# lpastura/kubernetes-1

Measured on AMD Instinct MI355X. Metric: pods scheduled/sec, higher is better.
Workload: dtype int64; 1 GPU; (b) 5000 nodes / 1913000 pods; nodes=5000, nodes_per_gpu=5000, pods=1913000, percentage_of_nodes_to_score=100, parallelism=1 GPU

## Files before the change

### kubernetes-1_amd/csrc/kgpu_kernels.hip

```cpp
#include <hip/hip_runtime.h>

#include <algorithm>
#include <map>
#include <mutex>
#include <tuple>

#include "kgpu_internal.h"

#if defined(__HIP_DEVICE_COMPILE__)
#define GAS __attribute__((address_space(1)))
#define CAS __attribute__((address_space(4)))
#else
#define GAS
#define CAS
#endif

namespace kgpu {

template <class T>
__device__ __forceinline__ GAS T* gp(T* p) {
  return (GAS T*)p;
}
template <class T>
__device__ __forceinline__ const CAS T* cp(const T* p) {
  return (const CAS T*)p;
}


constexpr uint32_t kRuntime = 0xFFFFFFFFu;
constexpr uint32_t kDefRes = 1u << 31;
constexpr uint32_t kSMask = (1u << KGPU_NUM_SCORES) - 1;

__device__ __forceinline__ uint64_t splitmix64(uint64_t x) {
  x += 0x9E3779B97F4A7C15ull;
  uint64_t z = x;
  z = (z ^ (z >> 30)) * 0xBF58476D1CE4E5B9ull;
  z = (z ^ (z >> 27)) * 0x94D049BB133111EBull;
  return z ^ (z >> 31);
}
__device__ __forceinline__ uint64_t pod_tie_key(uint64_t seed, int64_t seq) {
  return splitmix64(seed ^ ((uint64_t)seq * 0x9E3779B97F4A7C15ull));
}
__device__ __forceinline__ uint64_t rank40(uint64_t k, uint64_t idx, int mode) {
  if (mode == 1) return kMask40 - idx;
  uint64_t x = idx & kMask40;
  x ^= k & kMask40;
  x = (x * 0xD6E8FEB865ull) & kMask40;
  x ^= x >> 19;
  x = (x * 0x94D049BB13ull) & kMask40;
  x ^= x >> 23;
  x ^= (k >> 24) & kMask40;
  return x;
}

__device__ __forceinline__ uint64_t rank40_inv(uint64_t k, uint64_t x, int mode) {
  if (mode == 1) return kMask40 - x;
  x ^= (k >> 24) & kMask40;
  x ^= x >> 23;
  x = (x * 0x38E12D471Bull) & kMask40;
  x ^= (x >> 19) ^ (x >> 38);
  x = (x * 0xB38E39396Dull) & kMask40;
  x ^= k & kMask40;
  return x;
}

__device__ __forceinline__ bool list_has(const int32_t* v, int n, int x) {
  for (int i = 0; i < n; ++i)
    if (cp(v)[i] == x) return true;
  return false;
}

__device__ bool node_req(const DevState& st, const kgpu_req& r, int n) {
  const int v = r.key >= 0 ? gp(st.label_val)[(size_t)r.key * st.N + n] : -1;
  switch (r.op) {
    case KGPU_OP_IN:
      return v >= 0 && list_has(st.qp.ints + r.vals.begin, r.vals.count, v);
    case KGPU_OP_NOTIN:
      return v < 0 || !list_has(st.qp.ints + r.vals.begin, r.vals.count, v);
    case KGPU_OP_EXISTS:
      return v >= 0;
    case KGPU_OP_DNE:
      return v < 0;
    default: {
      if (v < 0) return false;
      const int idx = gp(st.value_off)[r.key] + v;
      if (!gp(st.value_int_ok)[idx]) return false;
      const int64_t lv = gp(st.value_int)[idx];
      return r.op == KGPU_OP_GT ? lv > r.imm : lv < r.imm;
    }
  }
}

__device__ bool node_reqs_all(const DevState& st, kgpu_range rr, int n) {
  for (int i = 0; i < rr.count; ++i)
    if (!node_req(st, cp(st.qp.reqs)[rr.begin + i], n)) return false;
  return true;
}

__device__ bool node_affinity_ok(const DevState& st, const kgpu_pod_query& q, int n) {
  if (!node_reqs_all(st, q.node_selector, n)) return false;
  if (!(q.flags & KGPU_Q_REQ_NODE_AFFINITY)) return true;
  const int g = st.node_base + n;
  for (int t = 0; t < q.req_terms.count; ++t) {
    const kgpu_node_term term = cp(st.qp.node_terms)[q.req_terms.begin + t];
    if (term.never_match) continue;
    if (!node_reqs_all(st, term.reqs, n)) continue;
    if (term.field_op == KGPU_OP_IN && g != term.field_node) continue;
    if (term.field_op == KGPU_OP_NOTIN && g == term.field_node) continue;
    return true;
  }
  return false;
}

struct NodeRes {
  int64_t ac, am, ae;
  int64_t rc, rm, re;
  int64_t zc, zm;
  int32_t ap, np;
  double ic, im;
};

__device__ __forceinline__ NodeRes load_res(const DevState& st, int n) {
  NodeRes r;
  r.ac = gp(st.alloc_cpu)[n]; r.am = gp(st.alloc_mem)[n]; r.ae = gp(st.alloc_eph)[n];
  r.rc = gp(st.req_cpu)[n]; r.rm = gp(st.req_mem)[n]; r.re = gp(st.req_eph)[n];
  r.zc = gp(st.nz_cpu)[n]; r.zm = gp(st.nz_mem)[n];
  r.ap = gp(st.alloc_pods)[n]; r.np = gp(st.num_pods)[n];
  r.ic = 0.0;
  r.im = 0.0;
  return r;
}

__device__ __forceinline__ void set_recips(NodeRes& r) {
  r.ic = (r.ac > 0 && r.ac < (1ll << 52)) ? 1.0 / (double)r.ac : 0.0;
  r.im = (r.am > 0 && r.am < (1ll << 52)) ? 1.0 / (double)r.am : 0.0;
}

__device__ __forceinline__ uint32_t fit_detail(const DevState& st, const kgpu_pod_query& q, const NodeRes& r, int n) {
  uint32_t d = 0;
  if (r.np + 1 > r.ap) d |= 1u;
  if (q.flags & KGPU_Q_FIT_ALL_ZERO) return d;
  if (r.ac < q.req[0] + r.rc) d |= 2u;
  if (r.am < q.req[1] + r.rm) d |= 4u;
  if (r.ae < q.req[2] + r.re) d |= 8u;
  for (int i = 0; i < q.scalars.count; ++i) {
    const kgpu_scalar_req s = cp(st.qp.scalars)[q.scalars.begin + i];
    if (!s.check) continue;
    const int64_t alloc = s.col >= 0 ? gp(st.alloc_scalar)[(size_t)s.col * st.N + n] : 0;
    const int64_t used = s.col >= 0 ? gp(st.req_scalar)[(size_t)s.col * st.N + n] : 0;
    if (alloc < s.value + used) d |= 16u << (i < 11 ? i : 11);
  }
  return d;
}

__device__ __forceinline__ bool ports_conflict(const DevState& st, const kgpu_pod_query& q, int n) {
  const int have = gp(st.port_count)[n];
  for (int i = 0; i < q.ports.count; ++i) {
    const kgpu_port w = cp(st.qp.ports)[q.ports.begin + i];
// ... 1042 lines not shown
        __hip_atomic_fetch_or(abort_word, kAbortDirty, __ATOMIC_RELAXED, __HIP_MEMORY_SCOPE_AGENT);
        return;
      }
    }
  }
}
__device__ __forceinline__ void lds_wait(int* f, int v, int32_t* abort_word) { lds_wait_t<false>(f, v, abort_word); }
__device__ __forceinline__ void lds_wait_ge(int* f, int v, int32_t* abort_word) { lds_wait_t<true>(f, v, abort_word); }

__device__ __forceinline__ constexpr bool spare_slot(int j, int K, int tid, int B) {
  return j == K - 1 && tid == B - 1;
}

template <int K, int B>
__device__ __forceinline__ void wg_partials(BatchShared<B>& sh, int p, const uint64_t (&keys)[K], bool vb, int ob,
                                            int jb, int cand, Cand& ra, Cand& rb) {
  const int tid = threadIdx.x, lane = tid & 63, wave = tid >> 6;
  Cand a{0, -1, 0}, b{0, -1, 0};
  if (!vb) {
#pragma unroll
    for (int j = 0; j < K; ++j) {
      const uint64_t k = spare_slot(j, K, tid, B) ? 0 : keys[j];
      a.feas += __popcll(__ballot(k != 0));
      if (k > a.key) { a.key = k; a.idx = j * B + tid; }
    }
    wave_argmax(a.key, a.idx);
  } else {
    uint64_t m = 0, kc = 0, ks = 0;
    int mi = -1, f0 = 0;
#pragma unroll
    for (int j = 0; j < K; ++j) {
      const bool spare = spare_slot(j, K, tid, B), isc = tid == ob && j == jb;
      const uint64_t k = (spare || isc) ? 0 : keys[j];
      f0 += __popcll(__ballot(k != 0));
      if (k > m) { m = k; mi = j * B + tid; }
      if (isc) kc = keys[j];
      if (spare) ks = keys[j];
    }
    wave_argmax(m, mi);
    const uint64_t kcu = (ob >> 6) == wave ? (uint64_t)lane64((int64_t)kc, ob & 63) : 0;
    const uint64_t ksu = ((B - 1) >> 6) == wave ? (uint64_t)lane64((int64_t)ks, (B - 1) & 63) : 0;
    a = Cand{m, mi, f0 + (kcu != 0 ? 1 : 0)};
    if (kcu > m) { a.key = kcu; a.idx = jb * B + ob; }
    b = Cand{m, mi, f0 + (ksu != 0 ? 1 : 0)};
    if (ksu > m) { b.key = ksu; b.idx = cand; }
  }
  if (lane == 0) {
    sh.ka[p][wave] = a.key; sh.ia[p][wave] = a.idx; sh.fa[p][wave] = a.feas;
    sh.kb[p][wave] = b.key; sh.ib[p][wave] = b.idx; sh.fb[p][wave] = b.feas;
  }
  ra = a;
  rb = b;
}

template <int B>
__device__ __forceinline__ Cand wg_combine(const BatchShared<B>& sh, int p, bool variant_b) {
  Cand c{0, -1, 0};
#pragma unroll
  for (int w = 0; w < B / 64; ++w) {
    const uint64_t k = variant_b ? sh.kb[p][w] : sh.ka[p][w];
    const int i = variant_b ? sh.ib[p][w] : sh.ia[p][w];
    c.feas += variant_b ? sh.fb[p][w] : sh.fa[p][w];
    if (k > c.key) { c.key = k; c.idx = i; }
  }
  return c;
}

template <int K, int B>
__device__ __forceinline__ Cand wave_recombine(const BatchShared<B>& sh, int p, const uint64_t (&keys)[K]) {
  const int tid = threadIdx.x, wave = tid >> 6;
  Cand a{0, -1, 0};
#pragma unroll
  for (int j = 0; j < K; ++j) {
    const uint64_t k = spare_slot(j, K, tid, B) ? 0 : keys[j];
    a.feas += __popcll(__ballot(k != 0));
    if (k > a.key) { a.key = k; a.idx = j * B + tid; }
  }
  wave_argmax(a.key, a.idx);
  Cand c{0, -1, 0};
#pragma unroll
  for (int w = 0; w < B / 64; ++w) {
    const bool me = w == wave;
    const uint64_t k = me ? a.key : sh.ka[p][w];
    const int i = me ? a.idx : sh.ia[p][w];
    c.feas += me ? a.feas : sh.fa[p][w];
    if (k > c.key) { c.key = k; c.idx = i; }
  }
  return c;
}

template <int NJ>
struct Sweep {
  uint64_t v[NJ];
  int abort;
};
template <int NJ, bool SYS>
__device__ __forceinline__ Sweep<NJ> sweep(const uint64_t* row, int G, const int32_t* abort_word, uint64_t fill) {
  const int lane = threadIdx.x & 63;
  Sweep<NJ> s;
#pragma unroll
  for (int j = 0; j < NJ; ++j) {
    uint64_t* p = const_cast<uint64_t*>(row + lane + 64 * j);
    s.v[j] = (lane + 64 * j < G) ? (SYS ? __hip_atomic_load(p, __ATOMIC_RELAXED, __HIP_MEMORY_SCOPE_SYSTEM) : load_sc1(p))
                                 : fill;
  }
  s.abort = load_sc1(abort_word);
  return s;
}

template <int NJ>
__device__ __forceinline__ bool row_done(const Sweep<NJ>& cur, uint64_t tmask, uint64_t expect, uint64_t& wkey,
                                         int& wg) {
  const int lane = threadIdx.x & 63;
  bool all = true;
  uint64_t k = 0;
  int gsel = -1;
#pragma unroll
  for (int j = 0; j < NJ; ++j) {
    const uint64_t v = cur.v[j];
    if ((v & tmask) != expect) {
      all = false;
    } else if ((v & ~tmask) > k) {
      k = v & ~tmask;
      gsel = lane + 64 * j;
    }
  }
  if (!__all(all)) return false;
  wave_argmax(k, gsel);
  wkey = k;
  wg = k ? gsel : -1;
  return true;
}
template <int NJ, bool SYS>
__device__ __forceinline__ bool poll_row(const uint64_t* row, int G, const int32_t* abort_word, uint64_t tmask,
                                         uint64_t expect, uint64_t& wkey, int& wg) {
  const uint64_t t0 = __builtin_amdgcn_s_memrealtime();
  Sweep<NJ> a = sweep<NJ, SYS>(row, G, abort_word, expect);
  for (;;) {
    const Sweep<NJ> b = sweep<NJ, SYS>(row, G, abort_word, expect);
    if (a.abort != 0) return false;
    if (row_done<NJ>(a, tmask, expect, wkey, wg)) return true;
    a = sweep<NJ, SYS>(row, G, abort_word, expect);
    if (b.abort != 0) return false;
    if (row_done<NJ>(b, tmask, expect, wkey, wg)) return true;
    if (__builtin_amdgcn_s_memrealtime() - t0 > kSpinTimeout) return false;
  }
}

struct HRow {
  int64_t ac, am, zc, zm;
  double ic, im;
};

template <uint32_t FM, uint32_t SM, int K, int B, bool XG, bool HB = false>
__global__ __launch_bounds__(B + 64 + (HB ? 2 * B : 0)) void k_batch(const DevState* __restrict__ stp, BatchArgs pa) {
  static_assert(!HB || (B == 64 && !XG &&
                       SM == ((1u << KGPU_S_BALANCED_ALLOCATION) | (1u << KGPU_S_LEAST_ALLOCATED) | kDefRes)),
                "the helper wave splits config (b)'s profile on the one-row-wave geometry");
  const DevState& st = *stp;
  constexpr int W = B / 64;
  const int tid = threadIdx.x, wave = tid >> 6, lane = tid & 63;
  const int G = gridDim.x, g = blockIdx.x;
  if (g == pa.hold) return;
  const int lo = g * pa.per;
  const int GT = pa.GT, gme = pa.rank * G + g;
  constexpr bool xg = XG;
  const uint64_t tmask = xg ? (0xFull << 60) : kGValid;
  __shared__ BatchShared<B> sh;
  __shared__ int64_t sh_hk[HB ? 2 * 2 * K * B : 1];
  __shared__ int sh_hready[2];
  __shared__ uint64_t* sh_peer_g[XG ? kMaxRanks : 1];
  __shared__ int32_t* sh_peer_f[XG ? kMaxRanks : 1];
  if constexpr (XG) {
    if (wave == W && lane < pa.nranks) {
      sh_peer_g[lane] = pa.pgran[lane];
      sh_peer_f[lane] = pa.pfeas[lane];
    }
  }
  if (tid == 0) {
    sh.bready = 0;
    sh.cready = 0;
    sh_hready[0] = 0;
    sh_hready[1] = 0;
  }
  __syncthreads();
  auto ring_row = [&](int k) -> size_t { return xg ? (size_t)((pa.xseq0 + k) % pa.R) : (size_t)k; };
  auto ring_tag = [&](int k) -> uint64_t {
    return xg ? (kGValid | ((uint64_t)(((pa.xseq0 + k) / pa.R) & 7) << 60)) : kGValid;
  };
  auto publish = [&](int i, uint64_t key, int feas) {
    const size_t roff = ring_row(i) * GT + gme;
    const uint64_t gtag = ring_tag(i);
    if constexpr (!XG) {
      store_sc1(pa.gran + roff, gtag | key);
      pa.feas[roff] = feas;
    } else {
      for (int rk = 0; rk < pa.nranks; ++rk) {
        __hip_atomic_store(sh_peer_g[rk] + roff, gtag | key, __ATOMIC_RELAXED, __HIP_MEMORY_SCOPE_SYSTEM);
        __hip_atomic_store(sh_peer_f[rk] + roff, feas, __ATOMIC_RELAXED, __HIP_MEMORY_SCOPE_SYSTEM);
      }
    }
  };
  const bool tr = pa.trace && (g == 0 || g == G - 1);
  int64_t* trow = pa.trace ? pa.trace + (g == 0 ? 0 : 8) : nullptr;
#define KGPU_STAMP(i, k) \
  if (tr && (tid == 0 || tid == B)) trow[(size_t)(i) * 16 + (k)] = (int64_t)__builtin_amdgcn_s_memrealtime()

  if constexpr (HB) {
    if (wave == W + 1 || wave == W + 2) {
      const int hw = wave - W - 1;
      HRow h[K];
#pragma unroll
      for (int j = 0; j < K; ++j) {
        const int n = lo + j * B + lane;
        h[j] = HRow{0, 0, 0, 0, 0.0, 0.0};
        if (!spare_slot(j, K, lane, B) && n < st.N) {
          h[j].ac = gp(st.alloc_cpu)[n];
          h[j].am = gp(st.alloc_mem)[n];
          h[j].zc = gp(st.nz_cpu)[n];
          h[j].zm = gp(st.nz_mem)[n];
          h[j].ic = (h[j].ac > 0 && h[j].ac < (1ll << 52)) ? 1.0 / (double)h[j].ac : 0.0;
          h[j].im = (h[j].am > 0 && h[j].am < (1ll << 52)) ? 1.0 / (double)h[j].am : 0.0;
        }
      }
      __builtin_amdgcn_s_waitcnt(0);
      const int64_t wl = st.w_of[KGPU_S_LEAST_ALLOCATED], wbal = st.w_of[KGPU_S_BALANCED_ALLOCATION];
      int cand = -1;
      bool staged = false;
      for (int i = 0; i <= pa.count; ++i) {
        const bool have_prev = i > 0, have_cur = i < pa.count;
        const int p = i & 1;
        const kgpu_pod_query* qc = st.queries + pa.first + i;
        const kgpu_pod_query* qpp = st.queries + pa.first + i - 1;
        const bool qmem = have_prev && (cp(qpp)->scalars.count | cp(qpp)->ports.count) != 0;
        const bool fast_b = have_prev && cand >= 0 && staged && pa.assume && !qmem;
        const int ob = cand >= 0 ? cand % B : -1, jb = cand >= 0 ? cand / B : -1;
        if (have_cur) {
          if (fast_b) {
            HRow t{};
#pragma unroll
            for (int j = 0; j < K; ++j)
              if (j == jb) {
                t.ac = lane64(h[j].ac, ob);
                t.am = lane64(h[j].am, ob);
                t.zc = lane64(h[j].zc, ob) + cp(qpp)->nz[0];
                t.zm = lane64(h[j].zm, ob) + cp(qpp)->nz[1];
                t.ic = __builtin_bit_cast(double, lane64(__builtin_bit_cast(int64_t, h[j].ic), ob));
                t.im = __builtin_bit_cast(double, lane64(__builtin_bit_cast(int64_t, h[j].im), ob));
              }
            if (lane == B - 1) h[K - 1] = t;
          }
          kgpu_pod_query qh;
          qh.score_req[0] = cp(qc)->score_req[0];
          qh.score_req[1] = cp(qc)->score_req[1];
#pragma unroll
          for (int j = 0; j < K; ++j) {
            const bool spare = spare_slot(j, K, lane, B);
            const int n = spare ? lo + cand : lo + j * B + lane;
            NodeRes nr{};
            nr.ac = h[j].ac; nr.am = h[j].am; nr.zc = h[j].zc; nr.zm = h[j].zm; nr.ic = h[j].ic; nr.im = h[j].im;
            sh_hk[((hw * 2 + p) * K + j) * B + lane] =
                hw == 0 ? least_score<true>(st, qh, nr, n) * wl : balanced_score(qh, nr) * wbal;
          }
          if (lane == 0) lds_release(&sh_hready[hw], i + 1);
        }
        __syncthreads();
        int wg = -1;
        if (have_prev) {
          if (sh.rabort[(i - 1) & 1]) break;
          wg = sh.rwg[(i - 1) & 1];
        }
        const bool won = have_prev && wg == gme;
        if (won && pa.assume && lane == ob) {
#pragma unroll
          for (int j = 0; j < K; ++j)
            if (j == jb) {
              h[j].zc += cp(qpp)->nz[0];
              h[j].zm += cp(qpp)->nz[1];
            }
        }
        const bool slow = have_cur && won && pa.assume && !fast_b;
        int cn = -1;
        if (have_cur && !slow) {
          const Cand c = wg_combine<B>(sh, p, won && fast_b);
          cn = c.key ? c.idx : -1;
        }
        if (slow) {
          lds_wait(&sh.cready, i + 1, pa.abort);
          cand = sh.cslow[p];
        } else {
          cand = cn;
        }
        staged = have_cur && !slow && cand >= 0;
      }
      return;
    }
  }
  if (wave == W) {
    constexpr int kQWords = (int)(sizeof(kgpu_pod_query) / 8);
    static_assert(kQWords <= 64, "one query row per prefetch instruction");
    int cand = -1;
    bool staged = false;
    for (int i = 0; i <= pa.count; ++i) {
      const bool have_prev = i > 0, have_cur = i < pa.count;
      const int p = i & 1;
      if (i == pa.abort_at && g == 0 && lane == 0) __hip_atomic_store(pa.abort, 1, __ATOMIC_RELAXED, __HIP_MEMORY_SCOPE_AGENT);
      if (i + 2 < pa.count) {
        const uint64_t v = lane < kQWords ? reinterpret_cast<const uint64_t*>(st.queries + pa.first + i + 2)[lane] : 0;
        asm volatile("" ::"v"(v));
      }
      bool qmem = false;
      if (have_prev) {
        const kgpu_pod_query* qq = st.queries + pa.first + i - 1;
        qmem = (cp(qq)->scalars.count | cp(qq)->ports.count) != 0;
      }
      const bool fast_b = have_prev && cand >= 0 && staged && pa.assume && !qmem;
      uint64_t wkey = 0;
      int wg = -1;
      bool ok = true;
      if (have_prev) {
        const uint64_t* prow = pa.gran + ring_row(i - 1) * GT;
        const uint64_t expect = ring_tag(i - 1);
        if constexpr (!XG)
          ok = poll_row<4, false>(prow, GT, pa.abort, tmask, expect, wkey, wg);
        else if (GT <= 256)
          ok = poll_row<4, true>(prow, GT, pa.abort, tmask, expect, wkey, wg);
        else
          ok = poll_row<16, true>(prow, GT, pa.abort, tmask, expect, wkey, wg);
        KGPU_STAMP(i, 7);
      }
      const bool won = have_prev && wg == gme;
      const bool slow = have_cur && won && pa.assume && !fast_b;
      if (ok) {
        if (have_prev && lane == 0 && (xg ? g == 0 : (won || (wg < 0 && g == 0)))) {
          kgpu_result res;
          res.node = wg < 0 ? -1
                   : xg ? (int32_t)rank40_inv(pod_tie_key(st.seed, pa.seq0 + i - 1), wkey & kMask40, st.tie_mode)
                        : st.node_base + lo + cand;
          res.feasible = 0;
          res.evaluated = st.n_total;
          res.scored = 0;
          res.score = wg >= 0 ? (int64_t)(wkey >> 40) - 1 : 0;
          gp(st.results)[pa.first + i - 1] = res;
        }
      } else if (lane == 0) {
        __hip_atomic_fetch_or(pa.abort, (i <= 1 && !XG) ? kAbortClean : kAbortDirty, __ATOMIC_RELAXED,
                              __HIP_MEMORY_SCOPE_AGENT);
      }
      if (lane == 0 && have_prev) {
        sh.rwg[(i - 1) & 1] = wg;
        sh.rabort[(i - 1) & 1] = ok ? 0 : 1;
      }
      __syncthreads();
      if (!ok) break;
      int cn = -1;
      if (have_cur && !slow) {
        KGPU_STAMP(i, 6);
        const Cand c = wg_combine<B>(sh, p, won && fast_b);
        if (lane == 0) publish(i, c.key, c.feas);
        KGPU_STAMP(i, 3);
        cn = c.key ? c.idx : -1;
      }
      if (slow) {
        lds_wait(&sh.cready, i + 1, pa.abort);
        cand = sh.cslow[p];
      } else {
        cand = cn;
      }
      staged = have_cur && !slow && cand >= 0;
    }
    return;
  }

  constexpr bool kStream = K > 4;
  constexpr int KR = kStream ? 1 : K;
  static_assert(!kStream || (W > 1 && !HB), "streamed rows: the candidate row travels through sh.brow");
  constexpr bool kRecip = (SM & kDefRes) != 0 && SM != kRuntime;
  NodeRes r[KR];
#pragma unroll
  for (int j = 0; j < KR; ++j) {
    const int n = lo + j * B + tid;
    r[j] = NodeRes{};
    if (!kStream && !spare_slot(j, K, tid, B) && n < st.N) r[j] = load_row<kRecip>(st, n);
  }
  __builtin_amdgcn_s_waitcnt(0);

  kgpu_pod_query qp{};
  kgpu_pod_query q = *cp(st.queries + pa.first);
  int cand = -1;
  bool staged = false;
  for (int i = 0; i <= pa.count; ++i) {
    KGPU_STAMP(i, 0);
    const bool have_prev = i > 0;
    const bool have_cur = i < pa.count;
    const int p = i & 1;
    const bool fast_b = have_prev && cand >= 0 && staged && pa.assume && qp.scalars.count == 0 && qp.ports.count == 0;
    const int ob = cand >= 0 ? cand % B : -1, jb = cand >= 0 ? cand / B : -1;
    uint64_t keys[K];
    Cand own_a{0, -1, 0}, own_b{0, -1, 0};
    if (have_cur) {
      const uint64_t tk = pod_tie_key(st.seed, pa.seq0 + i);
      if (fast_b && wave == W - 1) {
        NodeRes t;
        if constexpr (W == 1) {
#pragma unroll
          for (int j = 0; j < K; ++j)
            if (j == jb) t = lane_row(r[j], ob);
        } else {
          lds_wait(&sh.bready, i, pa.abort);
          t = sh.brow[(i - 1) & 1];
        }
        assume_regs(qp, t);
        if (tid == B - 1) r[KR - 1] = t;
      }
      if constexpr (HB) {
        uint32_t fs[K];
        uint64_t rkj[K];
#pragma unroll
        for (int j = 0; j < K; ++j) {
          const bool spare = spare_slot(j, K, tid, B);
          const int n = spare ? lo + cand : lo + j * B + tid;
          fs[j] = (spare ? fast_b : n < st.N) ? run_filters<FM>(st, q, r[j], n) : 1u;
          rkj[j] = rank40(tk, (uint64_t)(st.node_base + n), st.tie_mode);
        }
        if (q.scalars.count | q.ports.count) vm_drain();
        lds_wait_ge(&sh_hready[0], i + 1, pa.abort);
        lds_wait_ge(&sh_hready[1], i + 1, pa.abort);
#pragma unroll
        for (int j = 0; j < K; ++j) {
          const int64_t tot = sh_hk[((0 * 2 + p) * K + j) * B + tid] + sh_hk[((1 * 2 + p) * K + j) * B + tid];
          keys[j] = fs[j] ? 0 : (((uint64_t)(tot + 1) << 40) | rkj[j]);
        }
      } else {
#pragma unroll
        for (int j = 0; j < K; ++j) {
          const bool spare = spare_slot(j, K, tid, B);
          const int n = spare ? lo + cand : lo + j * B + tid;
          if constexpr (kStream) {
            const bool live = spare ? fast_b : n < st.N;
            NodeRes rj = r[0];
            if (!spare && live) rj = load_row<kRecip>(st, n);
            keys[j] = live ? node_key<FM, SM>(st, q, rj, n, tk) : 0;
          } else {
            keys[j] = (spare ? fast_b : n < st.N) ? node_key<FM, SM>(st, q, r[j], n, tk) : 0;
          }
        }
      }
      KGPU_STAMP(i, 5);
      wg_partials<K, B>(sh, p, keys, fast_b, ob, jb, cand, own_a, own_b);
    }
    KGPU_STAMP(i, 1);
    kgpu_pod_query qn{};
    if (i + 1 < pa.count) qn = *cp(st.queries + pa.first + i + 1);
    __syncthreads();
    KGPU_STAMP(i, 2);
    int wg = -1;
    if (have_prev) {
      const int s = (i - 1) & 1;
      if (sh.rabort[s]) break;
      wg = sh.rwg[s];
    }
    const bool won = have_prev && wg == gme;
    int cn = -1;
    if (have_cur) {
      if (won && pa.assume && !fast_b) {
        cn = -2;
      } else {
        const Cand c = W == 1 ? ((won && fast_b) ? own_b : own_a) : wg_combine<B>(sh, p, won && fast_b);
        cn = c.key ? c.idx : -1;
      }
    }
    if (won && pa.assume && tid == ob) {
#pragma unroll
      for (int j = 0; j < K; ++j)
        if (j == jb) {
          if constexpr (kStream) {
            NodeRes t = load_res(st, lo + (j * B + tid));
            assume_row(st, qp, t, lo + (j * B + tid));
          } else {
            assume_row(st, qp, r[j], lo + (j * B + tid));
          }
          assume_counts(st, pa.first + i - 1, lo + (j * B + tid));
        }
    }
    const bool slow = cn == -2;
    if (slow) {
      if (wave == ob / 64) {
        if (tid == ob) {
          const uint64_t tk = pod_tie_key(st.seed, pa.seq0 + i);
#pragma unroll
          for (int j = 0; j < K; ++j)
            if (j == jb) {
              if constexpr (kStream) keys[j] = node_key<FM, SM>(st, q, load_row<kRecip>(st, lo + (j * B + tid)), lo + (j * B + tid), tk);
              else keys[j] = node_key<FM, SM>(st, q, r[j], lo + (j * B + tid), tk);
            }
        }
        const Cand c = wave_recombine<K, B>(sh, p, keys);
        if (lane == 0) {
          publish(i, c.key, c.feas);
          sh.cslow[p] = c.key ? c.idx : -1;
          lds_release(&sh.cready, i + 1);
        }
      }
      lds_wait(&sh.cready, i + 1, pa.abort);
      cand = sh.cslow[p];
    } else {
      cand = cn;
      if (W > 1 && cand >= 0 && tid == cand % B) {
#pragma unroll
        for (int j = 0; j < K; ++j)
          if (j == cand / B) {
            if constexpr (kStream) sh.brow[p] = load_row<kRecip>(st, lo + cand);
            else sh.brow[p] = r[j];
          }
        if (i != pa.skip_release_at) lds_release(&sh.bready, i + 1);
      }
    }
    staged = have_cur && !slow && cand >= 0;
    qp = q;
    q = qn;
    KGPU_STAMP(i, 4);
  }
#undef KGPU_STAMP
}

__global__ __launch_bounds__(256) void k_batch_fixup(const DevState* __restrict__ stp, BatchArgs pa, int G) {
  const DevState& st = *stp;
  const int lane = threadIdx.x & 63;
  const int i = blockIdx.x * 4 + (threadIdx.x >> 6);
  for (int64_t z = (int64_t)blockIdx.x * blockDim.x + threadIdx.x; z < pa.zero_n16; z += (int64_t)gridDim.x * blockDim.x) {
    uint4* zp = reinterpret_cast<uint4*>(pa.zero_buf) + z;
    *zp = uint4{0, 0, 0, 0};
  }
  if (pa.abort_out && blockIdx.x == 0 && threadIdx.x == 0)
    __hip_atomic_store(pa.abort_out, load_sc1(pa.abort), __ATOMIC_RELAXED, __HIP_MEMORY_SCOPE_SYSTEM);
  if (i >= pa.count) return;
  const size_t row = pa.R > 0 ? (size_t)((pa.xseq0 + i) % pa.R) : (size_t)i;
  int f = 0;
  for (int g = lane; g < pa.GT; g += 64) f += pa.feas[row * pa.GT + g];
  f = (int)wave_sum32((uint32_t)f);
  (void)G;
  if (lane == 0) {
    kgpu_result& r = gp(st.results)[pa.first + i];
    r.feasible = f;
    if (r.node >= 0 && f >= 2) {
      r.scored = 1;
    } else {
      r.scored = 0;
      r.score = 0;
    }
    if (pa.res_out) pa.res_out[pa.first + i] = r;
  }
}

__device__ __forceinline__ int nval(const DevState& st, int k, int n) {
  return k >= 0 ? gp(st.label_val)[(size_t)k * st.N + n] : -1;
}
__device__ __forceinline__ int64_t* slot_ptr(const DevState& st, const QPlan& pl, int slot) {
  return st.scratch + pl.slot_off[slot];
}
__device__ __forceinline__ TopoHdr* hdr(const DevState& st) { return reinterpret_cast<TopoHdr*>(st.scratch); }
__device__ __forceinline__ int64_t* zone_sums(const DevState& st) { return st.scratch + kHdrWords; }
__device__ __forceinline__ void add64(int64_t* p, int64_t v) {
  atomicAdd(reinterpret_cast<unsigned long long*>(p), (unsigned long long)v);
}
__device__ __forceinline__ unsigned long long enc_max(int64_t x) { return (unsigned long long)x ^ (1ull << 63); }
__device__ __forceinline__ void amax64(int64_t* p, int64_t x) {
  atomicMax(reinterpret_cast<unsigned long long*>(p), enc_max(x));
}
__device__ __forceinline__ void amin64(int64_t* p, int64_t x) {
  atomicMax(reinterpret_cast<unsigned long long*>(p), ~enc_max(x));
}
__device__ __forceinline__ int64_t read_max(const int64_t* p) {
  const unsigned long long u = *reinterpret_cast<const unsigned long long*>(p);
  return u ? (int64_t)(u ^ (1ull << 63)) : INT64_MIN;
}
__device__ __forceinline__ int64_t read_min(const int64_t* p) {
  const unsigned long long u = *reinterpret_cast<const unsigned long long*>(p);
  return u ? (int64_t)(~u ^ (1ull << 63)) : INT64_MAX;
}

__device__ __forceinline__ bool all_keys(const DevState& st, const TSpread* c, int nc, int n) {
  for (int i = 0; i < nc; ++i)
    if (nval(st, c[i].key, n) < 0) return false;
  return true;
}

__device__ uint32_t topo_filter(int f, const DevState& st, const QPlan& pl, int n) {
  const TopoHdr* h = hdr(st);
  if (f == KGPU_F_POD_TOPOLOGY_SPREAD) {
    if (pl.n_hard == 0 || !h->pany) return 0;
    for (int i = 0; i < pl.n_hard; ++i) {
      const TSpread& c = pl.hard[i];
      const int v = nval(st, c.key, n);
      if (v < 0) return KGPU_CODE_UNSCHEDULABLE << 8;
      const int64_t match = slot_ptr(st, pl, c.rslot)[v] ? slot_ptr(st, pl, c.cslot)[v] : 0;
      int64_t mn = read_min(&h->pmin[i]);
      if (mn == INT64_MAX) mn = 2147483647;
      if (match + c.self_match - mn > c.max_skew) return KGPU_CODE_UNSCHEDULABLE << 8;
    }
    return 0;
  }
  if (f == KGPU_F_INTER_POD_AFFINITY) {
    bool exist = true;
    for (int i = 0; i < pl.n_aff; ++i) {
      const int v = nval(st, pl.aff[i].key, n);
      if (v < 0) return (KGPU_CODE_UNRESOLVABLE << 8) | (1u << 16);
      if (slot_ptr(st, pl, pl.aff[i].slot)[v] <= 0) exist = false;
    }
    if (!exist && !(!h->aff_any && pl.self_all)) return (KGPU_CODE_UNRESOLVABLE << 8) | (1u << 16);
    for (int i = 0; i < pl.n_anti; ++i) {
      const int v = nval(st, pl.anti[i].key, n);
      if (v >= 0 && slot_ptr(st, pl, pl.anti[i].slot)[v] > 0) return (KGPU_CODE_UNSCHEDULABLE << 8) | (2u << 16);
// ... 1869 lines not shown

constexpr uint32_t bit(int i) { return 1u << i; }
constexpr uint32_t kFitFM = bit(KGPU_F_NODE_RESOURCES_FIT);
constexpr uint32_t kFitSM = bit(KGPU_S_BALANCED_ALLOCATION) | bit(KGPU_S_LEAST_ALLOCATED) | kDefRes;
constexpr uint32_t kDefaultFM = (1u << KGPU_NUM_FILTERS) - 1;
constexpr uint32_t kProviderSM = (1u << (KGPU_S_MOST_ALLOCATED + 1)) - 1;
constexpr uint32_t kDefaultSM = (kProviderSM & ~bit(KGPU_S_MOST_ALLOCATED)) | kDefRes;
constexpr uint32_t kAutoscalerSM = (kProviderSM & ~bit(KGPU_S_LEAST_ALLOCATED)) | kDefRes;

struct TGeo {
  int B, K;
};
constexpr TGeo kTGeo[] = {{256, 1}, {512, 1}, {512, 2}, {512, 4}, {512, 8}};
constexpr int kNumTGeo = sizeof(kTGeo) / sizeof(kTGeo[0]);
using TBatchFn = void (*)(const DevState*, TBatchArgs);
template <uint32_t FM, uint32_t SM, bool kDef, bool XG>
struct TBatchRow {
  static constexpr TBatchFn fn[kNumTGeo] = {k_tbatch<256, 1, FM, SM, kDef, XG>, k_tbatch<512, 1, FM, SM, kDef, XG>,
                                            k_tbatch<512, 2, FM, SM, kDef, XG>, k_tbatch<512, 4, FM, SM, kDef, XG>,
                                            k_tbatch<512, 8, FM, SM, kDef, XG>};
};
static const TBatchFn* const kTBatch[2][4] = {
    {TBatchRow<kRuntime, kRuntime, false, false>::fn, TBatchRow<kRuntime, kRuntime, true, false>::fn,
     TBatchRow<kDefaultFM, kDefaultSM, true, false>::fn, TBatchRow<kDefaultFM, kAutoscalerSM, true, false>::fn},
    {TBatchRow<kRuntime, kRuntime, false, true>::fn, TBatchRow<kRuntime, kRuntime, true, true>::fn,
     TBatchRow<kDefaultFM, kDefaultSM, true, true>::fn, TBatchRow<kDefaultFM, kAutoscalerSM, true, true>::fn}};

int64_t kernel_layout_sig() { return layout_sig_of(); }

int tbatch_geometry(int N, int max_groups, int* per, int* groups, int first) {
  for (int gi = first < 0 ? 0 : first; gi < kNumTGeo; ++gi) {
    const int p = kTGeo[gi].B * kTGeo[gi].K;
    const int g = (N + p - 1) / p;
    if (g <= max_groups) {
      *per = p;
      *groups = g < 1 ? 1 : g;
      return gi;
    }
  }
  return -1;
}

static bool grid_fits(const void* fn, int threads, size_t lds, int groups) {
  static std::mutex mu;
  static std::map<std::tuple<const void*, int, size_t>, int> cap;
  std::lock_guard<std::mutex> lock(mu);
  auto key = std::make_tuple(fn, threads, lds);
  auto it = cap.find(key);
  if (it == cap.end()) {
    int per_cu = 0, dev = 0, cus = 0;
    if (hipOccupancyMaxActiveBlocksPerMultiprocessor(&per_cu, fn, threads, lds) != hipSuccess) per_cu = 0;
    if (hipGetDevice(&dev) != hipSuccess ||
        hipDeviceGetAttribute(&cus, hipDeviceAttributeMultiprocessorCount, dev) != hipSuccess)
      cus = 0;
    it = cap.emplace(key, per_cu * cus).first;
  }
  return groups <= it->second;
}

int launch_tbatch_init(const DevState* st, const TBatchArgs& a, int groups, void* stream) {
  hipStream_t s = (hipStream_t)stream;
  const int N = a.per * groups;
  const int nb = (N + 255) / 256;
  const int nlh = a.lds_bins + a.n_hists;
  if (nlh <= kInitLdsBins)
    hipLaunchKernelGGL(k_tbatch_init<true>, dim3(nb), dim3(256), (unsigned)(sizeof(int32_t) * (size_t)std::max(nlh, 1)), s, st, a);
  else
    hipLaunchKernelGGL(k_tbatch_init<false>, dim3(nb), dim3(256), 0, s, st, a);
  return hipGetLastError() == hipSuccess ? 0 : -1;
}

int tbatch_row(int spec, bool def_res) { return spec == 2 ? 2 : (spec == 3 ? 3 : (def_res ? 1 : 0)); }

int launch_tbatch(const DevState* st, const TBatchArgs& a, int groups, int geo, int spec, bool xg, bool coop,
                  void* stream) {
  if (geo < 0 || geo >= kNumTGeo) return -1;
  hipStream_t s = (hipStream_t)stream;
  const int row = tbatch_row(spec, a.def_res != 0);
  const TBatchFn fn = kTBatch[xg ? 1 : 0][row][geo];
  static bool attr[2][4][kNumTGeo] = {};
  if (!attr[xg ? 1 : 0][row][geo]) {
    if (hipFuncSetAttribute(reinterpret_cast<const void*>(fn), hipFuncAttributeMaxDynamicSharedMemorySize,
                            kTLdsBudget) != hipSuccess)
      return -1;
    attr[xg ? 1 : 0][row][geo] = true;
  }
  TBatchArgs arg = a;
  const DevState* sp = st;
  void* args[] = {(void*)&sp, (void*)&arg};
  if (!coop && grid_fits(reinterpret_cast<const void*>(fn), kTGeo[geo].B, (size_t)a.lds_bytes, groups)) {
    hipLaunchKernelGGL(fn, dim3(groups), dim3(kTGeo[geo].B), (unsigned)a.lds_bytes, s, sp, arg);
    return hipGetLastError() == hipSuccess ? 0 : -1;
  }
  arg.hold = -1;
  return hipLaunchCooperativeKernel(reinterpret_cast<const void*>(fn), dim3(groups), dim3(kTGeo[geo].B), args,
                                    (unsigned)a.lds_bytes, s) == hipSuccess
             ? 0
             : -1;
}

struct SpecEntry {
  uint32_t fm, sm;
  void (*fn)(const DevState*, PodArgs);
};
static const SpecEntry kSpecs[] = {
    {kRuntime, kRuntime, k_eval<kRuntime, kRuntime>},
    {kFitFM, kFitSM, k_eval<kFitFM, kFitSM>},
    {kDefaultFM, kDefaultSM, k_eval<kDefaultFM, kDefaultSM>},
    {kDefaultFM, kAutoscalerSM, k_eval<kDefaultFM, kAutoscalerSM>},
};
constexpr int kNumSpecs = sizeof(kSpecs) / sizeof(kSpecs[0]);

int select_spec(const int32_t* filters, int nf, const int32_t* scores, int ns, bool def_res) {
  uint32_t fm = 0, sm = 0;
  for (int i = 0; i < nf; ++i) {
    if (i > 0 && filters[i] <= filters[i - 1]) return 0;
    fm |= bit(filters[i]);
  }
  for (int i = 0; i < ns; ++i) sm |= bit(scores[i]);
  const bool uses_res = (sm & (bit(KGPU_S_LEAST_ALLOCATED) | bit(KGPU_S_MOST_ALLOCATED))) != 0;
  if (uses_res) {
    if (!def_res) return 0;
    sm |= kDefRes;
  }
  for (int s = 1; s < kNumSpecs; ++s) {
    const uint32_t want = kSpecs[s].sm & (uses_res ? ~0u : ~kDefRes);
    if (kSpecs[s].fm == fm && want == sm) return s;
  }
  return 0;
}

struct Geo {
  int B, K;
};
constexpr Geo kGeo[] = {{64, 1}, {128, 1}, {192, 1}, {448, 1}, {960, 1}, {512, 4}, {512, 8}};
constexpr int kNumGeo = sizeof(kGeo) / sizeof(kGeo[0]);
constexpr int kBatchLdsPad = 96 * 1024;

template <uint32_t FM, uint32_t SM>
struct BatchRow {
  using Fn = void (*)(const DevState*, BatchArgs);
  static constexpr Fn fn[kNumGeo] = {k_batch<FM, SM, 1, 64, false>,  k_batch<FM, SM, 1, 128, false>,
                                     k_batch<FM, SM, 1, 192, false>, k_batch<FM, SM, 1, 448, false>,
                                     k_batch<FM, SM, 1, 960, false>, k_batch<FM, SM, 4, 512, false>,
                                     k_batch<FM, SM, 8, 512, false>};
  static constexpr Fn xfn[kNumGeo] = {k_batch<FM, SM, 1, 64, true>,  k_batch<FM, SM, 1, 128, true>,
                                      k_batch<FM, SM, 1, 192, true>, k_batch<FM, SM, 1, 448, true>,
                                      k_batch<FM, SM, 1, 960, true>, k_batch<FM, SM, 4, 512, true>,
                                      k_batch<FM, SM, 8, 512, true>};
};
using BatchFn = void (*)(const DevState*, BatchArgs);
template <uint32_t FM, uint32_t SM, bool E>
struct HelperFn {
  static constexpr BatchFn fn = nullptr;
};
template <uint32_t FM, uint32_t SM>
struct HelperFn<FM, SM, true> {
  static constexpr BatchFn fn = k_batch<FM, SM, 1, 64, false, true>;
};
static const BatchFn kBatchHelper[] = {
    nullptr,
    HelperFn<kFitFM, kFitSM, true>::fn,
    nullptr,
    nullptr,
};
static const BatchFn* const kBatch[] = {
    BatchRow<kRuntime, kRuntime>::fn,
    BatchRow<kFitFM, kFitSM>::fn,
    BatchRow<kDefaultFM, kDefaultSM>::fn,
    BatchRow<kDefaultFM, kAutoscalerSM>::fn,
};
static_assert(sizeof(kBatch) / sizeof(kBatch[0]) == kNumSpecs, "one k_batch row per profile instantiation");
static const BatchFn* const kBatchX[] = {
    BatchRow<kRuntime, kRuntime>::xfn,
    BatchRow<kFitFM, kFitSM>::xfn,
    BatchRow<kDefaultFM, kDefaultSM>::xfn,
    BatchRow<kDefaultFM, kAutoscalerSM>::xfn,
};

int batch_geometry(int N, int max_groups, int* per, int* groups, int first) {
  for (int gi = first < 0 ? 0 : first; gi < kNumGeo; ++gi) {
    const int p = kGeo[gi].B * kGeo[gi].K - 1;
    const int g = (N + p - 1) / p;
    if (g <= max_groups) {
      *per = p;
      *groups = g < 1 ? 1 : g;
      return gi;
    }
  }
  return -1;
}

bool geometry_shape(int kernel, int geo, int* threads, int* rows) {
  if (kernel == 1 && geo >= 0 && geo < kNumGeo) {
    *threads = kGeo[geo].B;
    *rows = kGeo[geo].K;
    return true;
  }
  if (kernel == 2 && geo >= 0 && geo < kNumTGeo) {
    *threads = kTGeo[geo].B;
    *rows = kTGeo[geo].K;
    return true;
  }
  return false;
}

int batch_row(int spec) { return spec < 0 || spec >= kNumSpecs ? 0 : spec; }

bool batch_helper_used(int spec, int geo, bool sharded, bool helper) {
  return helper && !sharded && geo == 0 && kBatchHelper[batch_row(spec)] != nullptr;
}

int launch_batch(const DevState* st, const BatchArgs& a, int groups, int geo, int spec, bool coop, bool helper,
                 void* stream) {
  spec = batch_row(spec);
  if (geo < 0 || geo >= kNumGeo) return -1;
  const int x = a.R > 0 ? 1 : 0;
  const bool hb = batch_helper_used(spec, geo, x != 0, helper);
  const BatchFn fn = hb ? kBatchHelper[spec] : (x ? kBatchX : kBatch)[spec][geo];
  const int threads = kGeo[geo].B + 64 + (hb ? 2 * kGeo[geo].B : 0);
  static bool attr_set[3][kNumSpecs][kNumGeo] = {};
  const int ai = hb ? 2 : x;
  if (!attr_set[ai][spec][geo]) {
    if (hipFuncSetAttribute(reinterpret_cast<const void*>(fn), hipFuncAttributeMaxDynamicSharedMemorySize,
                            kBatchLdsPad) != hipSuccess)
      return -1;
    attr_set[ai][spec][geo] = true;
  }
  BatchArgs arg = a;
  const DevState* sp = st;
  void* args[] = {(void*)&sp, (void*)&arg};
  if (!coop && grid_fits(reinterpret_cast<const void*>(fn), threads, (size_t)kBatchLdsPad, groups)) {
    hipLaunchKernelGGL(fn, dim3(groups), dim3(threads), (unsigned)kBatchLdsPad, (hipStream_t)stream, sp, arg);
    if (hipGetLastError() != hipSuccess) return -1;
  } else {
    arg.hold = -1;
    if (hipLaunchCooperativeKernel(reinterpret_cast<const void*>(fn), dim3(groups), dim3(threads), args,
                                   (unsigned)kBatchLdsPad, (hipStream_t)stream) != hipSuccess)
      return -1;
  }
  hipLaunchKernelGGL(k_batch_fixup, dim3((a.count + 3) / 4), dim3(256), 0, (hipStream_t)stream, st, a, groups);
  return hipGetLastError() == hipSuccess ? 0 : -1;
}

int eval_blocks(int N) {
  int b = (N + kBlock - 1) / kBlock;
  if (b > kMaxBlocks) b = kMaxBlocks;
  if (b < 1) b = 1;
  return b;
}

int launch_eval(const DevState* st, const PodArgs& a, int blocks, int spec, void* stream) {
  if (spec < 0 || spec >= kNumSpecs) spec = 0;
  hipLaunchKernelGGL(kSpecs[spec].fn, dim3(blocks), dim3(kBlock), 0, (hipStream_t)stream, st, a);
  return hipGetLastError() == hipSuccess ? 0 : -1;
}

int launch_final(const DevState* st, const PodArgs& a, int blocks, int stat_blocks, void* stream) {
  hipLaunchKernelGGL(k_final, dim3(blocks), dim3(kBlock), 0, (hipStream_t)stream, st, a, stat_blocks);
  return hipGetLastError() == hipSuccess ? 0 : -1;
}

int launch_cut(const DevState* st, const PodArgs& a, int blocks, int n_filters, void* stream) {
  hipLaunchKernelGGL(k_cut, dim3(1), dim3(kCutThreads), 0, (hipStream_t)stream, st, a, blocks, n_filters);
  return hipGetLastError() == hipSuccess ? 0 : -1;
}

int launch_resolve(const DevState* st, int N, const PodArgs& a, void* stream) {
  hipLaunchKernelGGL(k_resolve, dim3(eval_blocks(N)), dim3(kBlock), 0, (hipStream_t)stream, st, a);
  return hipGetLastError() == hipSuccess ? 0 : -1;
}

int launch_shard_pack(const DevState* st, int parity, int blocks, int what, void* stream) {
  hipLaunchKernelGGL(k_shard_pack, dim3(1), dim3(kBlock), 0, (hipStream_t)stream, st, parity, blocks, what);
  return hipGetLastError() == hipSuccess ? 0 : -1;
}

__global__ __launch_bounds__(kBlock) void k_delta(const DevState* __restrict__ stp, DeltaArgs a) {
  const DevState& st = *stp;
  const int lane = threadIdx.x;
  const size_t N = (size_t)st.N;
  const int o0 = a.group_off[blockIdx.x], o1 = a.group_off[blockIdx.x + 1];
  for (int o = o0; o < o1; ++o) {
    const DeltaOp op = a.ops[o];
    const int n = op.node;
    if (op.kind == kDSetNode) {
      const kgpu_node_row r = a.rows[op.item];
      if (lane == 0) {
        gp(st.alloc_cpu)[n] = r.alloc_cpu;
        gp(st.alloc_mem)[n] = r.alloc_mem;
        gp(st.alloc_eph)[n] = r.alloc_eph;
        gp(st.alloc_pods)[n] = r.alloc_pods;
        gp(st.unsched)[n] = (uint8_t)(r.unschedulable ? 1 : 0);
        gp(st.zone_id)[n] = r.zone_id;
      }
      for (int k = lane; k < st.K; k += kBlock) {
        int32_t v = -1;
        for (int j = 0; j + 1 < r.labels.count; j += 2)
          if (a.ints[r.labels.begin + j] == k) v = a.ints[r.labels.begin + j + 1];
        gp(st.label_val)[(size_t)k * N + n] = v;
      }
      for (int w = lane; w < st.TW; w += kBlock) {
        const bool has = r.taints.count >= 2 * st.TW;
        gp(st.taint_nosched)[(size_t)w * N + n] = has ? a.words[r.taints.begin + w] : 0ull;
        gp(st.taint_prefer)[(size_t)w * N + n] = has ? a.words[r.taints.begin + st.TW + w] : 0ull;
      }
      for (int sc = lane; sc < st.S; sc += kBlock)
        gp(st.alloc_scalar)[(size_t)sc * N + n] =
            sc < r.alloc_scalar.count ? (int64_t)a.words[r.alloc_scalar.begin + sc] : 0;
    } else {
      const kgpu_pod_query q = a.pods[op.item];
      const int64_t sg = op.kind == kDAddPod ? 1 : -1;
      if (lane == 0) {
        gp(st.req_cpu)[n] += sg * q.req[0];
        gp(st.req_mem)[n] += sg * q.req[1];
        gp(st.req_eph)[n] += sg * q.req[2];
        gp(st.nz_cpu)[n] += sg * q.nz[0];
        gp(st.nz_mem)[n] += sg * q.nz[1];
        gp(st.num_pods)[n] += (int32_t)sg;
        for (int i = 0; i < q.scalars.count; ++i) {
          const kgpu_scalar_req sr = a.scalars[q.scalars.begin + i];
          if (sr.col >= 0) gp(st.req_scalar)[(size_t)sr.col * N + n] += sg * sr.value;
        }
        int pc = gp(st.port_count)[n];
        for (int i = 0; i < q.ports.count; ++i) {
          const kgpu_port w = a.ports[q.ports.begin + i];
          int at = -1;
          for (int s = 0; s < pc; ++s) {
            const kgpu_port p = gp(st.ports)[(size_t)s * N + n];
            if (p.ip == w.ip && p.proto == w.proto && p.port == w.port) at = s;
          }
          if (sg > 0) {
            if (at >= 0) continue;
            if (pc >= st.PS) {
              gp(st.port_overflow)[0] = 1;
              continue;
            }
            gp(st.ports)[(size_t)(pc++) * N + n] = w;
          } else if (at >= 0) {
            gp(st.ports)[(size_t)at * N + n] = gp(st.ports)[(size_t)(pc - 1) * N + n];
            --pc;
          }
        }
        gp(st.port_count)[n] = pc;
      }
      for (int i = lane; i < op.cls.count; i += kBlock)
        gp(st.mcnt)[(size_t)a.aux[op.cls.begin + i] * N + n] += (int32_t)sg;
      for (int i = lane; i < op.tcls.count; i += kBlock)
        gp(st.tcnt)[(size_t)a.aux[op.tcls.begin + i] * N + n] += (int32_t)sg;
    }
    __syncthreads();
  }
}

int launch_delta(const DevState* st, const DeltaArgs& a, void* stream) {
  if (a.n_ops <= 0 || a.n_groups <= 0) return 0;
  hipLaunchKernelGGL(k_delta, dim3(a.n_groups), dim3(kBlock), 0, (hipStream_t)stream, st, a);
  return hipGetLastError() == hipSuccess ? 0 : -1;
}

__global__ void k_remap(const RemapCol* __restrict__ cols, const int32_t* __restrict__ from, int old_n, int new_n) {
  const RemapCol c = cols[blockIdx.y];
  const size_t total = (size_t)c.ncols * (size_t)new_n;
  for (size_t e = (size_t)blockIdx.x * blockDim.x + threadIdx.x; e < total; e += (size_t)gridDim.x * blockDim.x) {
    const size_t col = e / (size_t)new_n, i = e - col * (size_t)new_n;
    const int f = from[i];
    const size_t so = col * (size_t)old_n + (size_t)(f < 0 ? 0 : f);
    switch (c.elem) {
      case 1: gp((uint8_t*)c.dst)[e] = f < 0 ? 0 : cp((const uint8_t*)c.src)[so]; break;
      case 4: gp((int32_t*)c.dst)[e] = f < 0 ? 0 : cp((const int32_t*)c.src)[so]; break;
      case 8: gp((int64_t*)c.dst)[e] = f < 0 ? 0 : cp((const int64_t*)c.src)[so]; break;
      default: {
        const kgpu_port z{0, 0, 0, 0};
        gp((kgpu_port*)c.dst)[e] = f < 0 ? z : cp((const kgpu_port*)c.src)[so];
      }
// ... 465 lines not shown
```

Measured before the change: 673,000 pods/s.

## Stage pod queries through an LDS ring in the helper-wave batch kernel

In the helper-wave k_batch instantiation, the control wave now prefetches each pod query three iterations ahead into a 4-entry shared-memory ring. Scoring, helper and control waves read the query from LDS with readfirstlane uniformization instead of issuing global/constant loads on the per-pod critical path. Trace stamps are compiled out of the helper kernel, and a separate traced twin is selected only when tracing is on. The cost is extra LDS, register pressure from holding the ring copies, and reliance on the ring write happening before the barrier at which consumers read it.

```diff
diff --git a/kubernetes-1_amd/csrc/kgpu_kernels.hip b/kubernetes-1_amd/csrc/kgpu_kernels.hip
--- a/kubernetes-1_amd/csrc/kgpu_kernels.hip
+++ b/kubernetes-1_amd/csrc/kgpu_kernels.hip
@@ -4,6 +4,7 @@
 #include <map>
 #include <mutex>
 #include <tuple>
+#include <type_traits>
 
 #include "kgpu_internal.h"
 
@@ -1352,11 +1353,37 @@
   double ic, im;
 };
 
-template <uint32_t FM, uint32_t SM, int K, int B, bool XG, bool HB = false>
+constexpr int kQRing = 4;
+constexpr int kQWords = (int)(sizeof(kgpu_pod_query) / 8);
+static_assert(kQWords <= 64, "one query row per vector load");
+typedef uint64_t __attribute__((may_alias)) qword_t;
+struct NoQuery {};
+__device__ __forceinline__ kgpu_pod_query ring_read(const kgpu_pod_query* ring, int k) {
+  const kgpu_pod_query& s = ring[k & (kQRing - 1)];
+  kgpu_pod_query q{};
+  q.flags = s.flags;
+  q.req[0] = s.req[0]; q.req[1] = s.req[1]; q.req[2] = s.req[2];
+  q.nz[0] = s.nz[0]; q.nz[1] = s.nz[1];
+  q.score_req[0] = s.score_req[0]; q.score_req[1] = s.score_req[1];
+  q.scalars = s.scalars;
+  q.ports = s.ports;
+  return q;
+}
+__device__ __forceinline__ kgpu_pod_query ring_uniform(kgpu_pod_query q) {
+  q.flags = __builtin_amdgcn_readfirstlane(q.flags);
+  q.scalars.begin = __builtin_amdgcn_readfirstlane(q.scalars.begin);
+  q.scalars.count = __builtin_amdgcn_readfirstlane(q.scalars.count);
+  q.ports.begin = __builtin_amdgcn_readfirstlane(q.ports.begin);
+  q.ports.count = __builtin_amdgcn_readfirstlane(q.ports.count);
+  return q;
+}
+
+template <uint32_t FM, uint32_t SM, int K, int B, bool XG, bool HB = false, bool TR = false>
 __global__ __launch_bounds__(B + 64 + (HB ? 2 * B : 0)) void k_batch(const DevState* __restrict__ stp, BatchArgs pa) {
   static_assert(!HB || (B == 64 && !XG &&
                        SM == ((1u << KGPU_S_BALANCED_ALLOCATION) | (1u << KGPU_S_LEAST_ALLOCATED) | kDefRes)),
                 "the helper wave splits config (b)'s profile on the one-row-wave geometry");
+  static_assert(HB || !TR, "only the helper-wave instantiation has a traced twin");
   const DevState& st = *stp;
   constexpr int W = B / 64;
   const int tid = threadIdx.x, wave = tid >> 6, lane = tid & 63;
@@ -1369,6 +1396,7 @@
   __shared__ BatchShared<B> sh;
   __shared__ int64_t sh_hk[HB ? 2 * 2 * K * B : 1];
   __shared__ int sh_hready[2];
+  __shared__ std::conditional_t<HB, kgpu_pod_query, NoQuery> sh_q[HB ? kQRing : 1];
   __shared__ uint64_t* sh_peer_g[XG ? kMaxRanks : 1];
   __shared__ int32_t* sh_peer_f[XG ? kMaxRanks : 1];
   if constexpr (XG) {
@@ -1382,6 +1410,11 @@
     sh.cready = 0;
     sh_hready[0] = 0;
     sh_hready[1] = 0;
+  }
+  if constexpr (HB) {
+    if (wave == W && lane < kQWords)
+      for (int k = 0; k < 3 && k < pa.count; ++k)
+        reinterpret_cast<qword_t*>(&sh_q[k])[lane] = ((const GAS qword_t*)(st.queries + pa.first + k))[lane];
   }
   __syncthreads();
   auto ring_row = [&](int k) -> size_t { return xg ? (size_t)((pa.xseq0 + k) % pa.R) : (size_t)k; };
@@ -1403,8 +1436,9 @@
   };
   const bool tr = pa.trace && (g == 0 || g == G - 1);
   int64_t* trow = pa.trace ? pa.trace + (g == 0 ? 0 : 8) : nullptr;
+  constexpr bool kStamps = !HB || TR;
 #define KGPU_STAMP(i, k) \
-  if (tr && (tid == 0 || tid == B)) trow[(size_t)(i) * 16 + (k)] = (int64_t)__builtin_amdgcn_s_memrealtime()
+  if (kStamps && tr && (tid == 0 || tid == B)) trow[(size_t)(i) * 16 + (k)] = (int64_t)__builtin_amdgcn_s_memrealtime()
 
   if constexpr (HB) {
     if (wave == W + 1 || wave == W + 2) {
@@ -1427,12 +1461,12 @@
       const int64_t wl = st.w_of[KGPU_S_LEAST_ALLOCATED], wbal = st.w_of[KGPU_S_BALANCED_ALLOCATION];
       int cand = -1;
       bool staged = false;
+      kgpu_pod_query rq = ring_uniform(ring_read(sh_q, 0)), rqp{};
       for (int i = 0; i <= pa.count; ++i) {
         const bool have_prev = i > 0, have_cur = i < pa.count;
         const int p = i & 1;
-        const kgpu_pod_query* qc = st.queries + pa.first + i;
-        const kgpu_pod_query* qpp = st.queries + pa.first + i - 1;
-        const bool qmem = have_prev && (cp(qpp)->scalars.count | cp(qpp)->ports.count) != 0;
+        const kgpu_pod_query rqn = ring_read(sh_q, i + 1);
+        const bool qmem = have_prev && (rqp.scalars.count | rqp.ports.count) != 0;
         const bool fast_b = have_prev && cand >= 0 && staged && pa.assume && !qmem;
         const int ob = cand >= 0 ? cand % B : -1, jb = cand >= 0 ? cand / B : -1;
         if (have_cur) {
@@ -1443,16 +1477,16 @@
               if (j == jb) {
                 t.ac = lane64(h[j].ac, ob);
                 t.am = lane64(h[j].am, ob);
-                t.zc = lane64(h[j].zc, ob) + cp(qpp)->nz[0];
-                t.zm = lane64(h[j].zm, ob) + cp(qpp)->nz[1];
+                t.zc = lane64(h[j].zc, ob) + rqp.nz[0];
+                t.zm = lane64(h[j].zm, ob) + rqp.nz[1];
                 t.ic = __builtin_bit_cast(double, lane64(__builtin_bit_cast(int64_t, h[j].ic), ob));
                 t.im = __builtin_bit_cast(double, lane64(__builtin_bit_cast(int64_t, h[j].im), ob));
               }
             if (lane == B - 1) h[K - 1] = t;
           }
           kgpu_pod_query qh;
-          qh.score_req[0] = cp(qc)->score_req[0];
-          qh.score_req[1] = cp(qc)->score_req[1];
+          qh.score_req[0] = rq.score_req[0];
+          qh.score_req[1] = rq.score_req[1];
 #pragma unroll
           for (int j = 0; j < K; ++j) {
             const bool spare = spare_slot(j, K, lane, B);
@@ -1475,10 +1509,12 @@
 #pragma unroll
           for (int j = 0; j < K; ++j)
             if (j == jb) {
-              h[j].zc += cp(qpp)->nz[0];
-              h[j].zm += cp(qpp)->nz[1];
+              h[j].zc += rqp.nz[0];
+              h[j].zm += rqp.nz[1];
             }
         }
+        rqp = rq;
+        rq = ring_uniform(rqn);
         const bool slow = have_cur && won && pa.assume && !fast_b;
         int cn = -1;
         if (have_cur && !slow) {
@@ -1497,22 +1533,28 @@
     }
   }
   if (wave == W) {
-    constexpr int kQWords = (int)(sizeof(kgpu_pod_query) / 8);
-    static_assert(kQWords <= 64, "one query row per prefetch instruction");
     int cand = -1;
     bool staged = false;
     for (int i = 0; i <= pa.count; ++i) {
       const bool have_prev = i > 0, have_cur = i < pa.count;
       const int p = i & 1;
       if (i == pa.abort_at && g == 0 && lane == 0) __hip_atomic_store(pa.abort, 1, __ATOMIC_RELAXED, __HIP_MEMORY_SCOPE_AGENT);
-      if (i + 2 < pa.count) {
+      uint64_t qv = 0;
+      if constexpr (HB) {
+        if (i + 3 < pa.count && lane < kQWords) qv = ((const GAS qword_t*)(st.queries + pa.first + i + 3))[lane];
+      } else if (i + 2 < pa.count) {
         const uint64_t v = lane < kQWords ? reinterpret_cast<const uint64_t*>(st.queries + pa.first + i + 2)[lane] : 0;
         asm volatile("" ::"v"(v));
       }
       bool qmem = false;
       if (have_prev) {
-        const kgpu_pod_query* qq = st.queries + pa.first + i - 1;
-        qmem = (cp(qq)->scalars.count | cp(qq)->ports.count) != 0;
+        if constexpr (HB) {
+          const kgpu_pod_query& qq = sh_q[(i - 1) & (kQRing - 1)];
+          qmem = __builtin_amdgcn_readfirstlane(qq.scalars.count | qq.ports.count) != 0;
+        } else {
+          const kgpu_pod_query* qq = st.queries + pa.first + i - 1;
+          qmem = (cp(qq)->scalars.count | cp(qq)->ports.count) != 0;
+        }
       }
       const bool fast_b = have_prev && cand >= 0 && staged && pa.assume && !qmem;
       uint64_t wkey = 0;
@@ -1561,6 +1603,9 @@
         KGPU_STAMP(i, 3);
         cn = c.key ? c.idx : -1;
       }
+      if constexpr (HB) {
+        if (i + 3 < pa.count && lane < kQWords) reinterpret_cast<qword_t*>(&sh_q[(i + 3) & (kQRing - 1)])[lane] = qv;
+      }
       if (slow) {
         lds_wait(&sh.cready, i + 1, pa.abort);
         cand = sh.cslow[p];
@@ -1587,10 +1632,13 @@
 
   kgpu_pod_query qp{};
   kgpu_pod_query q = *cp(st.queries + pa.first);
+  if constexpr (HB) q = ring_uniform(ring_read(sh_q, 0));
   int cand = -1;
   bool staged = false;
   for (int i = 0; i <= pa.count; ++i) {
     KGPU_STAMP(i, 0);
+    std::conditional_t<HB, kgpu_pod_query, NoQuery> qraw{};
+    if constexpr (HB) qraw = ring_read(sh_q, i + 1);
     const bool have_prev = i > 0;
     const bool have_cur = i < pa.count;
     const int p = i & 1;
@@ -1651,7 +1699,9 @@
     }
     KGPU_STAMP(i, 1);
     kgpu_pod_query qn{};
-    if (i + 1 < pa.count) qn = *cp(st.queries + pa.first + i + 1);
+    if constexpr (!HB) {
+      if (i + 1 < pa.count) qn = *cp(st.queries + pa.first + i + 1);
+    }
     __syncthreads();
     KGPU_STAMP(i, 2);
     int wg = -1;
@@ -1659,6 +1709,9 @@
       const int s = (i - 1) & 1;
       if (sh.rabort[s]) break;
       wg = sh.rwg[s];
+    }
+    if constexpr (HB) {
+      if (i + 1 < pa.count) qn = ring_uniform(qraw);
     }
     const bool won = have_prev && wg == gme;
     int cn = -1;
@@ -3834,15 +3887,22 @@
 using BatchFn = void (*)(const DevState*, BatchArgs);
 template <uint32_t FM, uint32_t SM, bool E>
 struct HelperFn {
-  static constexpr BatchFn fn = nullptr;
+  static constexpr BatchFn fn = nullptr, traced = nullptr;
 };
 template <uint32_t FM, uint32_t SM>
 struct HelperFn<FM, SM, true> {
   static constexpr BatchFn fn = k_batch<FM, SM, 1, 64, false, true>;
+  static constexpr BatchFn traced = k_batch<FM, SM, 1, 64, false, true, true>;
 };
 static const BatchFn kBatchHelper[] = {
     nullptr,
     HelperFn<kFitFM, kFitSM, true>::fn,
+    nullptr,
+    nullptr,
+};
+static const BatchFn kBatchHelperTraced[] = {
+    nullptr,
+    HelperFn<kFitFM, kFitSM, true>::traced,
     nullptr,
     nullptr,
 };
@@ -3899,10 +3959,11 @@
   if (geo < 0 || geo >= kNumGeo) return -1;
   const int x = a.R > 0 ? 1 : 0;
   const bool hb = batch_helper_used(spec, geo, x != 0, helper);
-  const BatchFn fn = hb ? kBatchHelper[spec] : (x ? kBatchX : kBatch)[spec][geo];
+  const bool traced = hb && a.trace != nullptr;
+  const BatchFn fn = hb ? (traced ? kBatchHelperTraced : kBatchHelper)[spec] : (x ? kBatchX : kBatch)[spec][geo];
   const int threads = kGeo[geo].B + 64 + (hb ? 2 * kGeo[geo].B : 0);
-  static bool attr_set[3][kNumSpecs][kNumGeo] = {};
-  const int ai = hb ? 2 : x;
+  static bool attr_set[4][kNumSpecs][kNumGeo] = {};
+  const int ai = hb ? (traced ? 3 : 2) : x;
   if (!attr_set[ai][spec][geo]) {
     if (hipFuncSetAttribute(reinterpret_cast<const void*>(fn), hipFuncAttributeMaxDynamicSharedMemorySize,
                             kBatchLdsPad) != hipSuccess)
```

Result: faster. 681,000 pods/s, median of 6 (+1.2%).
